# achiever04/face-recognition-platform

Hardware: AMD Instinct MI355X
Metric: faces/sec (detect+embed+match) on 1080p @ 100k gallery (higher is better)
Workload: dtype f16; 1 GPU; 32x1080x1920 BGR frames per GPU per step resident in HBM, host results out every step, 2 batches in flight per GPU (one handle = one stream each, used round-robin), forced K=10 faces/frame, 100000-identity fp16 gallery, FRPDet detector fp16 + ArcFace IResNet-100 fp16 (synthetic seeded weights); batch_frames=32, faces_per_frame=10, gallery=100000, streams=1, lanes=2, lane_warmup_steps=20

## Files before the change

face-recognition-platform_amd/csrc/conv_mfma.hip:

```cpp
#include <hip/hip_runtime.h>
#include <stdint.h>
#include <stdlib.h>
#include <type_traits>
#include "frp_internal.h"
#include "conv_common.h"

namespace frp {

template <int TP, int TC, int WP, int WC, int NS, int NW, bool SMALL>
__global__ __launch_bounds__(NW * 64, TP == 128 ? 4 : 2) void conv_mfma_kernel(ConvParams p_in) {
    extern __shared__ __attribute__((aligned(16))) unsigned char smem[];
    ConvParams p = p_in;
    if (p.n_dev) {
        int n = *p.n_dev;
        n = n < 0 ? 0 : (n > p.N ? p.N : n);
        p.M = n * p.Ho * p.Wo;
        p.n_ptiles = (p.M + TP - 1) / TP;
        if (p.ksplit < 0) p.ksplit = conv_pick_ksplit(p.M, p.Cout, p.Ktot, p.flags, p.res != nullptr, p.n_cu);
    }
    constexpr int XB = TP * 128;
    constexpr int WB = TC * 128;
    constexpr int STAGE = XB + WB;
    constexpr int XI = TP / 8 / NW;
    constexpr int WI = TC / 8 / NW;
// ... 340 lines not shown
        attr_set[dev] = true;
    }
    const int ncu = device_cu_count(dev);
    if (ncu <= 0) return hipErrorInvalidDevice;
    const int ks_grid = p.ksplit < 0 ? conv_pick_ksplit(p.Ho * p.Wo, p.Cout, p.Ktot, p.flags, p.res != nullptr, ncu) : p.ksplit;
    const long ntiles = (long)p.n_ptiles * p.n_ctiles * ks_grid;
    if (ntiles <= 0 || ntiles > 0x7fffffffL) return hipErrorInvalidValue;
    p.n_cu = ncu;
    const long slots = (long)ncu * (lds <= 80 * 1024 ? 2 : 1);
    unsigned grid = (unsigned)(ntiles < slots ? ntiles : slots);
    p.n_workers = 0;
    if (TP == 128 && p.pf_ptr && p.pf_bytes >= 4096 && grid <= 128 && (long)grid + CONV_PF_WGS <= slots) {
        p.n_workers = (int)grid;
        grid += CONV_PF_WGS;
    }
    if (grid > 256) p.stamps = nullptr;
    hipLaunchKernelGGL(kern, dim3(grid), dim3(NW * 64), lds, stream, p);
    return hipGetLastError();
}

hipError_t launch_conv(const ConvParams& in, hipStream_t stream) {
    ConvParams p = in;
    if (!(p.KS == 1 || p.KS == 3) || !(p.stride == 1 || p.stride == 2)) return hipErrorInvalidValue;
    if (p.Cin < 8 || (p.Cin & 7) || (p.Cout & 7) || p.N <= 0 || p.H <= 0 || p.W <= 0) return hipErrorInvalidValue;
    p.pad = p.KS / 2;
    p.Ho = (p.H + 2 * p.pad - p.KS) / p.stride + 1;
    p.Wo = (p.W + 2 * p.pad - p.KS) / p.stride + 1;
    const long M = (long)p.N * p.Ho * p.Wo;
    if (M <= 0 || M > 0x7fffffffL) return hipErrorInvalidValue;
    p.M = (int)M;
    p.Ktot = p.KS * p.KS * p.Cin;
    p.x2_bytes = 0;
    p.x2_shift = 0;
    if (p.x2) {
        if (p.KS != 3 || (p.Cin & 63) || p.Cin2 <= 0 || (p.Cin2 & 63) || !(p.Cin == p.Cin2 || p.Cin == 2 * p.Cin2) || p.ksplit > 1 ||
            (p.flags & (FRP_FLAG_F8 | FRP_FLAG_BORDER_BIAS)) || p.wino_w)
            return hipErrorInvalidValue;
        const long x2b = (long)p.N * p.H * p.W * p.Cin2 * 2;
        if (x2b >= 0x7fffffffL) return hipErrorInvalidValue;
        p.x2_bytes = (unsigned)x2b;
        p.x2_shift = p.Cin == p.Cin2 ? 0 : 1;
        p.Ktot += p.Cin2;
    }
    p.nk = (p.Ktot + 63) / 64;
    if (p.ksplit < 0 && !(p.n_dev && (p.flags & FRP_FLAG_OUT_F32) && !p.res && !(p.Cin & 63))) return hipErrorInvalidValue;
    if (p.ksplit == 0) p.ksplit = 1;
    if (p.ksplit > 1 && (p.nk % p.ksplit != 0 || !(p.flags & FRP_FLAG_OUT_F32) || p.res || (p.Cin & 63)))
        return hipErrorInvalidValue;
    const bool f8 = (p.flags & FRP_FLAG_F8) != 0;
    const int es = f8 ? 1 : 2;
    const long xb = (long)p.N * p.H * p.W * p.Cin * es, wb = (long)p.Cout * p.Ktot * es;
    if (xb >= 0x7fffffffL || wb >= 0x7fffffffL) return hipErrorInvalidValue;
    if ((p.flags & FRP_FLAG_OUT_FP8) && !f8) return hipErrorInvalidValue;
    if ((p.out2 || f8) && ((p.flags & FRP_FLAG_OUT_F32) || p.ksplit != 1 || !(p.out_scale > 0.f))) return hipErrorInvalidValue;
    p.x_bytes = (unsigned)xb;
    p.w_bytes = (unsigned)wb;
    const bool small = (p.Cin & 63) != 0;
    p.cin_shift = 0;
    if (small) {
        if (p.Cin & (p.Cin - 1)) return hipErrorInvalidValue;
        while ((1 << p.cin_shift) < p.Cin) ++p.cin_shift;
    }
    if ((p.flags & FRP_FLAG_BORDER_BIAS) && !(p.KS == 3 && p.stride == 1 && p.Ho >= 2 && p.Wo >= 2))
        return hipErrorInvalidValue;
    if ((p.flags & FRP_FLAG_RES_UP2) && (!p.res || p.Hr * 2 != p.Ho || p.Wr * 2 != p.Wo)) return hipErrorInvalidValue;
    if (!p.x || !p.w || !p.bias || !p.out) return hipErrorInvalidValue;
    if (p.act == FRP_ACT_PRELU && !p.slope) return hipErrorInvalidValue;
    if (f8) {
        if (!conv3x3_rows_eligible(p) || (p.Cin & 127) || !p.wscale || !(p.in_scale > 0.f)) return hipErrorInvalidValue;
        return launch_conv3x3_lean(p, stream);
    }
    int ncu_ = p.n_cu;
    if (ncu_ <= 0) {
        int dev_ = 0;
        if (hipGetDevice(&dev_) != hipSuccess || dev_ < 0 || dev_ >= 64) return hipErrorInvalidDevice;
        ncu_ = device_cu_count(dev_);
    }
    const bool few = conv_small_m(p, (long)((p.M + 255) / 256) * ((p.Cout + 127) / 128), ncu_);
    if (p.wino_w && !p.x2 && !(p.dbg & CONV_DBG_GENERIC) && conv3x3_wino_eligible(p)) {
        p.w = p.wino_w;
        return launch_conv3x3_wino(p, stream);
    }
    if ((p.dbg & CONV_DBG_S2) && !(p.dbg & CONV_DBG_GENERIC) && !few && conv3x3_s2_eligible(p)) return launch_conv3x3_s2(p, stream);
    if (p.stem_x) return (p.small_m <= 0 && conv3x3_c64_eligible(p)) ? launch_conv3x3_c64(p, stream) : hipErrorInvalidValue;
    if (!(p.dbg & (CONV_DBG_GENERIC | CONV_DBG_NO_C64)) && p.small_m <= 0 && conv3x3_c64_eligible(p)) return launch_conv3x3_c64(p, stream);
#ifdef FRP_LAB
    if (!(p.dbg & CONV_DBG_GENERIC) && !p.x2 && conv3x3_rows_eligible(p)) return launch_conv3x3_rows(p, stream);
#else
    if (!(p.dbg & CONV_DBG_GENERIC) && !p.x2 && conv3x3_rows_eligible(p)) return launch_conv3x3_lean(p, stream);
#endif
    if (!small && few) return launch_cfg<128, 64, 4, 2, 3, 8, false>(p, stream);
    if (p.Cout > 64)
        return small ? launch_cfg<256, 128, 4, 2, 3, 8, true>(p, stream) : launch_cfg<256, 128, 4, 2, 3, 8, false>(p, stream);
    return small ? launch_cfg<256, 64, 8, 1, 3, 8, true>(p, stream) : launch_cfg<256, 64, 8, 1, 3, 8, false>(p, stream);
}

}
```

face-recognition-platform_amd/csrc/frp_api.cpp:

```cpp
#include <hip/hip_runtime.h>
#include <rccl/rccl.h>
#include <dlfcn.h>

#include <algorithm>
#include <cmath>
#include <cstdio>
#include <cstdlib>
#include <cstring>
#include <mutex>
#include <string>
#include <vector>
#include <thread>
#include <atomic>

#include "frp.h"
#ifdef FRP_LAB
#include "frp_lab.h"
#endif
#include "frp_blob.h"
#include "frp_internal.h"
#include "jpeg_host.h"

using namespace frp;

#define FRP_WINO_MIN_FACES 128
Switches frp::read_switches() {
    auto set = [](const char* n) { return getenv(n) ? 1 : 0; };
    const char *sm = getenv("FRP_SMALL_M"), *wm = getenv("FRP_WINO_MIN_FACES");
    Switches s{};
    s.small_m = !sm ? 0 : (sm[0] == '0' ? -1 : 1);
    s.wino_min_faces = wm ? atoi(wm) : FRP_WINO_MIN_FACES;
    s.s2 = set("FRP_S2"); s.host_count = set("FRP_HOST_COUNT"); s.match_v1 = set("FRP_MATCH_V1");
    s.no_fused_stem12 = set("FRP_NO_FUSED_STEM12"); s.no_fused_stem = set("FRP_NO_FUSED_STEM");
    s.no_emb_stem = set("FRP_NO_EMB_STEM"); s.no_stem_fuse = set("FRP_NO_STEM_FUSE");
    s.no_wino = set("FRP_NO_WINO"); s.no_kconcat = set("FRP_NO_KCONCAT");
    return s;
}

const ProcessSwitches& frp::process_switches() {
    static const ProcessSwitches s = [] {
        const char* jh = getenv("FRP_JPEG_DEVICE_HUFFMAN");
        return ProcessSwitches{getenv("FRP_NO_GRAPH") != nullptr, getenv("FRP_C64_ALL") != nullptr, !jh ? 0 : (jh[0] == '0' ? -1 : 1)};
    }();
    return s;
}

namespace {

struct DevBuf {
    void* p = nullptr;
    size_t cap = 0;
};

struct TensorDims {
    int h = 0, w = 0, c = 0;
    bool f32 = false;
    bool f8 = false;
};

struct Net {
    std::vector<frp_conv_op> ops;
    int n_bufs = 0;
    int in_buf = 0, in_ch = 0;
    std::vector<DevBuf> bufs;
    std::vector<TensorDims> dims;
    std::vector<int64_t> wino_off;
    std::vector<int> kc_skip;
    std::vector<int> kc_src;
    std::vector<int64_t> kc_w_off, kc_bias_off;
};

enum { EV_START = 0, EV_H2D, EV_PRE, EV_DET, EV_DEC, EV_ALIGN, EV_EMB, EV_L2, EV_MATCH, EV_D2H, EV_COUNT };

struct NetGraph {
    std::string key;
    hipGraphExec_t exec = nullptr;
    uint64_t epoch = 0;
    double dflops = 0, df8flops = 0;
    int64_t dlaunches = 0, df8launches = 0;
    int fc_ksplit = 0, fc_ktot = 0;
    const float* fc_bias = nullptr;
    std::vector<TensorDims> dims;
};

}

struct frp_handle {
    int device = 0;
    hipStream_t stream = nullptr;
    std::mutex mu;
    std::string err;
    frp_config cfg{};
    bool have_weights = false;
    frp_blob_header hdr{};
    DevBuf wdata;
    Net det, emb;
    DevBuf frames;
    int rB = 0, rH = 0, rW = 0;
    int n_cu = 256;
    DevBuf frames_next;
    int nB = 0, nH = 0, nW = 0;
    bool next_valid = false;
    hipStream_t copy_stream = nullptr;
    hipEvent_t ev_next_ready = nullptr, ev_next_free = nullptr;
    std::vector<void*> pinned;
    DevBuf scaled;
    int dH = 0, dW = 0;
    bool det_scaled = false;
    int canvas_h = 0, canvas_w = 0;
    int det_op_limit = -1;
    std::vector<NetGraph> graphs;
    std::vector<std::string> graph_seen, graph_bad;
    uint64_t alloc_epoch = 1;
    int64_t graph_replays = 0;
    void* comm = nullptr;
    int dist_rank = 0, dist_world = 0;
    DevBuf det_hashes;
    bool det_hash_on = false;
// ... 175 lines not shown
    return (float)std::log((double)t / (1.0 - (double)t));
}

void rec(frp_handle* h, int which) {
    if (h->cfg.profile) (void)hipEventRecord(h->ev[which], h->stream);
}

int plan_net(frp_handle* h, Net& net, int batch, int H, int W, bool skip_input = false) {
    net.dims.assign(net.n_bufs, TensorDims());
    std::vector<size_t> need(net.n_bufs, 0);
    net.dims[net.in_buf] = {H, W, net.in_ch, false};
    need[net.in_buf] = skip_input ? 0 : (size_t)batch * H * W * net.in_ch * 2;
    for (const frp_conv_op& op : net.ops) {
        TensorDims in = net.dims[op.in_buf];
        if (in.c == 0) return fail(h, FRP_ERR_BLOB, "program reads an unwritten buffer");
        if (op.flags & FRP_FLAG_FLATTEN) in = {1, 1, in.h * in.w * in.c, false};
        if (in.c != op.cin) return fail(h, FRP_ERR_BLOB, "program channel mismatch");
        const int pad = op.ksize / 2;
        TensorDims out;
        out.h = (in.h + 2 * pad - op.ksize) / op.stride + 1;
        out.w = (in.w + 2 * pad - op.ksize) / op.stride + 1;
        out.c = op.cout;
        out.f32 = (op.flags & FRP_FLAG_OUT_F32) != 0;
        if (out.h <= 0 || out.w <= 0) return fail(h, FRP_ERR_INVALID, "input too small for the network");
        if (in.f32) return fail(h, FRP_ERR_BLOB, "program reads an fp32 tensor as a conv input");
        const bool op_f8 = (op.flags & FRP_OPFLAG_FP8_MFMA) != 0;
        if (in.f8 != op_f8) return fail(h, FRP_ERR_BLOB, "program operand precision mismatch (fp8 op <-> fp8 tensor)");
        if (op_f8 && !(op.ksize == 3 && op.stride == 1 && (op.cin & 127) == 0 && !(op.flags & (FRP_FLAG_OUT_F32 | FRP_FLAG_FLATTEN | FRP_FLAG_RES_UP2))))
            return fail(h, FRP_ERR_BLOB, "op shape not covered by the fp8 matrix path");
        out.f8 = (op.flags & FRP_OPFLAG_OUT_FP8) != 0;
        if (out.f8 && (out.f32 || !op_f8)) return fail(h, FRP_ERR_BLOB, "fp8 primary output needs an fp8 op");
        if (op.res_buf >= 0) {
            const TensorDims& r = net.dims[op.res_buf];
            const bool up2 = (op.flags & FRP_FLAG_RES_UP2) != 0;
            if (r.c != op.cout || r.f32 || r.f8 || (up2 ? (r.h * 2 != out.h || r.w * 2 != out.w) : (r.h != out.h || r.w != out.w)))
                return fail(h, FRP_ERR_BLOB, "program residual shape mismatch");
        }
        net.dims[op.out_buf] = out;
        need[op.out_buf] = std::max(need[op.out_buf], (size_t)batch * out.h * out.w * out.c * (out.f32 ? 4 : out.f8 ? 1 : 2));
        if (op.out2_buf >= 0) {
            if (out.f32 || out.f8) return fail(h, FRP_ERR_BLOB, "fp8 copy of a non-fp16 output");
            TensorDims o2 = out;
            o2.f8 = true;
            net.dims[op.out2_buf] = o2;
            need[op.out2_buf] = std::max(need[op.out2_buf], (size_t)batch * out.h * out.w * out.c);
        }
    }
    for (int i = 0; i < net.n_bufs; ++i)
        if (need[i]) FRPCHK(ensure(h, net.bufs[i], need[i]));
    return FRP_OK;
}

bool stem_fusable(const Net& net) {
    if (net.ops.empty()) return false;
    const frp_conv_op& op = net.ops[0];
    return op.in_buf == net.in_buf && op.cin == 8 && op.cout == 32 && op.ksize == 3 && op.stride == 2 &&
           op.act == FRP_ACT_RELU && op.res_buf < 0 && (op.flags & ~0) == 0 && (op.real_ch & 0xffff) == 3;
}

bool stem12_fusable(const Net& net) {
    if (!stem_fusable(net) || net.ops.size() < 2) return false;
    const frp_conv_op& a = net.ops[0];
    const frp_conv_op& b = net.ops[1];
    if (!(b.in_buf == a.out_buf && b.cin == 32 && b.cout == 64 && b.ksize == 3 && b.stride == 2 && b.act == FRP_ACT_RELU &&
          b.res_buf < 0 && b.flags == 0))
        return false;
    for (size_t i = 2; i < net.ops.size(); ++i)
        if (net.ops[i].in_buf == a.out_buf || net.ops[i].res_buf == a.out_buf) {
            bool rewritten = false;
            for (size_t j = 2; j < i; ++j) rewritten |= net.ops[j].out_buf == a.out_buf;
            if (!rewritten) return false;
        }
    return true;
}

int run_net_body(frp_handle* h, const Switches& sw, Net& net, int batch, int H, int W, double* flops, int64_t* launches, const StemParams* stem,
                 const int32_t* n_dev, bool allow_wino) {
    std::vector<TensorDims> d(net.n_bufs);
    d[net.in_buf] = {H, W, net.in_ch, false};
    const char* wbase = (const char*)h->wdata.p;
    bool first = true;
    size_t skip = 0;
    if (&net == &h->det && h->det_hash_on) HIPCHK(h, hipMemsetAsync(h->det_hashes.p, 0, 64 * 8, h->stream));
    const int dbg = (sw.s2 ? CONV_DBG_S2 : 0) | (process_switches().c64_all ? CONV_DBG_C64_ALL : 0);
    if (stem && stem12_fusable(net) && (stem->Hc % 4) == 0 && (stem->Wc % 4) == 0 && !sw.no_fused_stem12) {
        const frp_conv_op& a = net.ops[0];
        const frp_conv_op& b = net.ops[1];
        Stem12Params sp{};
        sp.frames = stem->frames; sp.B = stem->B; sp.H = stem->H; sp.W = stem->W;
        sp.row_stride = stem->row_stride; sp.frame_stride = stem->frame_stride;
        sp.Hc = stem->Hc; sp.Wc = stem->Wc; sp.Ho1 = stem->Hc / 2; sp.Wo1 = stem->Wc / 2; sp.Ho2 = stem->Hc / 4; sp.Wo2 = stem->Wc / 4;
        sp.rgb_in = stem->rgb_in;
        sp.w1 = (const _Float16*)(wbase + a.w_off); sp.bias1 = (const float*)(wbase + a.bias_off);
        sp.w2 = (const _Float16*)(wbase + b.w_off); sp.bias2 = (const float*)(wbase + b.bias_off);
        sp.out = (_Float16*)net.bufs[b.out_buf].p;
        hipError_t e = launch_stem12_u8(sp, h->stream);
        if (e != hipSuccess) return fail(h, FRP_ERR_HIP, std::string("launch_stem12_u8: ") + hipGetErrorString(e));
        d[a.out_buf] = {sp.Ho1, sp.Wo1, 32, false};
        d[b.out_buf] = {sp.Ho2, sp.Wo2, 64, false};
        *flops += 2.0 * batch * sp.Ho1 * sp.Wo1 * 9.0 * 3 * 32 + 2.0 * batch * sp.Ho2 * sp.Wo2 * 9.0 * 32 * 64;
        *launches += 1;
        if (h->det_hash_on) {
            e = launch_tensor_hash(sp.out, (size_t)batch * sp.Ho2 * sp.Wo2 * 64 * 2, (unsigned long long*)h->det_hashes.p + 1, h->stream);
            if (e != hipSuccess) return fail(h, FRP_ERR_HIP, std::string("tensor_hash: ") + hipGetErrorString(e));
        }
        skip = 2;
        first = false;
    }
    bool fuse_stem = false, fuse_even_only = false;
    size_t fuse_op = 0;
    EmbStemParams fused{};
    if (!stem && !net.ops.empty()) {
        const frp_conv_op& a = net.ops[0];
        if (a.in_buf == net.in_buf && a.cin == 8 && (a.real_ch & 0xffff) == 3 && a.cout == 64 && a.ksize == 3 && a.stride == 1 &&
            a.act == FRP_ACT_PRELU && a.res_buf < 0 && a.flags == 0 && a.slope_off >= 0 && !sw.no_emb_stem) {
            EmbStemParams ep{};
            ep.x = (const _Float16*)net.bufs[a.in_buf].p;
            ep.M = batch; ep.H = H; ep.W = W;
            ep.w = (const _Float16*)(wbase + a.w_off);
            ep.bias = (const float*)(wbase + a.bias_off);
            ep.slope = (const float*)(wbase + a.slope_off);
            ep.out = (_Float16*)net.bufs[a.out_buf].p;
            ep.n_dev = n_dev;
            size_t nb = 1;
            while (nb < net.ops.size() && nb < net.kc_skip.size() && net.kc_skip[nb]) ++nb;
            if (nb < net.ops.size() && !sw.no_stem_fuse && sw.small_m <= 0) {
                const frp_conv_op& b = net.ops[nb];
                const bool plain = !(b.flags & ~FRP_FLAG_BORDER_BIAS) && (b.flags & FRP_FLAG_BORDER_BIAS) && b.out2_buf < 0 && b.res_buf < 0;
                const bool chained = !(nb < net.kc_src.size() && net.kc_src[nb] >= 0);
                fuse_stem = plain && chained && b.in_buf == a.out_buf && b.out_buf != a.out_buf && b.out_buf != a.in_buf && a.out_buf != a.in_buf && b.cin == 64 && b.cout == 64 && b.ksize == 3 &&
                            b.stride == 1 && b.act == FRP_ACT_PRELU && b.slope_off >= 0 && conv3x3_c64_fuses_stem(batch, H, W, h->n_cu);
                fuse_op = nb;
                fuse_even_only = true;
                for (size_t j = 1; j < net.ops.size(); ++j) {
                    const frp_conv_op& o = net.ops[j];
                    if (j == nb || (o.in_buf != a.out_buf && o.res_buf != a.out_buf)) continue;
                    const bool shortcut = j < net.kc_skip.size() && net.kc_skip[j] && o.in_buf == a.out_buf && o.res_buf != a.out_buf &&
                                          o.ksize == 1 && o.stride == 2;
                    if (!shortcut) fuse_even_only = false;
                }
            }
            if (fuse_stem) {
                fused = ep;
            } else {
                hipError_t e = launch_emb_stem(ep, h->stream);
                if (e != hipSuccess) return fail(h, FRP_ERR_HIP, std::string("launch_emb_stem: ") + hipGetErrorString(e));
                *launches += 1;
            }
            d[a.out_buf] = {H, W, 64, false};
            *flops += 2.0 * batch * H * W * 9.0 * 3 * 64;
            skip = 1;
            first = false;
        }
    }
    for (const frp_conv_op& op : net.ops) {
        if (&net == &h->det && h->det_op_limit >= 0 && (int)(&op - net.ops.data()) >= h->det_op_limit) break;
        if (skip) { --skip; continue; }
        if (first && stem) {
            first = false;
            StemParams sp = *stem;
            sp.w = (const _Float16*)(wbase + op.w_off);
            sp.bias = (const float*)(wbase + op.bias_off);
            sp.out = (_Float16*)net.bufs[op.out_buf].p;
            hipError_t e = launch_stem_u8(sp, h->stream);
            if (e != hipSuccess) return fail(h, FRP_ERR_HIP, std::string("launch_stem_u8: ") + hipGetErrorString(e));
            d[op.out_buf] = {sp.Ho, sp.Wo, 32, false};
            *flops += 2.0 * batch * sp.Ho * sp.Wo * 9.0 * 3 * 32;
// ... 1745 lines not shown
    HIPCHK(h, hipMemcpyAsync(h->scratch.p, chips, (size_t)M * FRP_CHIP_PIX * 3, hipMemcpyHostToDevice, h->stream));
    hipError_t e = launch_chips_to_blob((const uint8_t*)h->scratch.p, M, (_Float16*)h->emb.bufs[h->emb.in_buf].p, h->stream);
    if (e != hipSuccess) return fail(h, FRP_ERR_HIP, std::string("chips_to_blob: ") + hipGetErrorString(e));
    FRPCHK(run_embed(h, read_switches(), M));
    HIPCHK(h, hipMemcpyAsync(emb, h->emb.bufs[h->hdr.emb_out_buf].p, (size_t)M * FRP_EMB_DIM * 4, hipMemcpyDeviceToHost, h->stream));
    HIPCHK(h, hipStreamSynchronize(h->stream));
    return FRP_OK;
}

static int match_common(frp_handle* h, const float* q, int M, float* all_scores_host, int32_t* idx, float* cos) {
    const Switches sw = read_switches();
    if (!q || M <= 0 || M > (1 << 20)) return fail(h, FRP_ERR_INVALID, "bad query arguments");
    if (h->g_rows <= 0) return fail(h, FRP_ERR_NO_GALLERY, "gallery is empty");
    const int mpad = round_up(M, 32);
    FRPCHK(ensure(h, h->q16, (size_t)mpad * FRP_EMB_DIM * 2));
    HIPCHK(h, hipMemsetAsync(h->q16.p, 0, (size_t)mpad * FRP_EMB_DIM * 2, h->stream));
    FRPCHK(upload_rows_normalized(h, q, M, (_Float16*)h->q16.p));
    DevBuf all;
    if (all_scores_host) FRPCHK(ensure(h, all, (size_t)M * h->g_rows * 4));
    int rc = run_match(h, sw, M, (float*)all.p);
    hipError_t e = hipSuccess;
    if (rc == FRP_OK) {
        if (idx) e = hipMemcpyAsync(idx, h->best_idx.p, (size_t)M * 4, hipMemcpyDeviceToHost, h->stream);
        if (e == hipSuccess && cos) e = hipMemcpyAsync(cos, h->best_cos.p, (size_t)M * 4, hipMemcpyDeviceToHost, h->stream);
        if (e == hipSuccess && all_scores_host)
            e = hipMemcpyAsync(all_scores_host, all.p, (size_t)M * h->g_rows * 4, hipMemcpyDeviceToHost, h->stream);
    }
    hipError_t e2 = hipStreamSynchronize(h->stream);
    release(all);
    if (rc != FRP_OK) return rc;
    if (e != hipSuccess || e2 != hipSuccess) return fail(h, FRP_ERR_HIP, "match result copy failed");
    return FRP_OK;
}

int frp_match(frp_handle* h, const float* q, int32_t M, int32_t topk, int32_t* idx, float* cos) {
    if (!h) return FRP_ERR_INVALID;
    Guard g(h);
    if (topk < 1 || topk > FRP_MAX_TOPK) return fail(h, FRP_ERR_INVALID, "topk must be in 1..FRP_MAX_TOPK");
    if (topk == 1) return match_common(h, q, M, nullptr, idx, cos);
    if (!q || !idx || !cos || M <= 0 || M > (1 << 20)) return fail(h, FRP_ERR_INVALID, "bad query arguments");
    if (h->g_rows <= 0) return fail(h, FRP_ERR_NO_GALLERY, "gallery is empty");
    const long N = h->g_rows;
    const Switches sw = read_switches();
    int chunk = (int)std::max<long>(1, std::min<long>(M, (1L << 28) / N));
    DevBuf all, didx, dcos;
    int rc = ensure(h, all, (size_t)chunk * N * 4);
    if (rc == FRP_OK) rc = ensure(h, didx, (size_t)chunk * topk * 4);
    if (rc == FRP_OK) rc = ensure(h, dcos, (size_t)chunk * topk * 4);
    hipError_t e = hipSuccess;
    for (int m0 = 0; rc == FRP_OK && e == hipSuccess && m0 < M; m0 += chunk) {
        const int m = std::min(chunk, M - m0);
        const int mpad = round_up(m, 32);
        rc = ensure(h, h->q16, (size_t)mpad * FRP_EMB_DIM * 2);
        if (rc != FRP_OK) break;
        e = hipMemsetAsync(h->q16.p, 0, (size_t)mpad * FRP_EMB_DIM * 2, h->stream);
        if (e != hipSuccess) break;
        rc = upload_rows_normalized(h, q + (size_t)m0 * FRP_EMB_DIM, m, (_Float16*)h->q16.p);
        if (rc == FRP_OK) rc = run_match(h, sw, m, (float*)all.p);
        if (rc != FRP_OK) break;
        e = launch_topk_rows((const float*)all.p, m, N, topk, (int32_t*)didx.p, (float*)dcos.p, h->stream);
        if (e == hipSuccess) e = hipMemcpyAsync(idx + (size_t)m0 * topk, didx.p, (size_t)m * topk * 4, hipMemcpyDeviceToHost, h->stream);
        if (e == hipSuccess) e = hipMemcpyAsync(cos + (size_t)m0 * topk, dcos.p, (size_t)m * topk * 4, hipMemcpyDeviceToHost, h->stream);
        if (e == hipSuccess) e = hipStreamSynchronize(h->stream);
    }
    (void)hipStreamSynchronize(h->stream);
    release(all); release(didx); release(dcos);
    if (rc != FRP_OK) return rc;
    if (e != hipSuccess) return fail(h, FRP_ERR_HIP, std::string("match top-k: ") + hipGetErrorString(e));
    return FRP_OK;
}

int frp_match_scores(frp_handle* h, const float* q, int32_t M, float* cos_all, int64_t n_cols) {
    if (!h) return FRP_ERR_INVALID;
    Guard g(h);
    if (!cos_all) return fail(h, FRP_ERR_INVALID, "null output");
    if (n_cols != h->g_rows) return fail(h, FRP_ERR_INVALID, "match_scores: output sized for another gallery size");
    return match_common(h, q, M, cos_all, nullptr, nullptr);
}

namespace {
void conv_route_from_abi_flags(int32_t flags, ConvParams& p) {
    p.dbg = ((flags >> 8) & 0xff) | ((flags & (1 << 19)) ? CONV_DBG_WINO_2D : 0) | ((flags & (1 << 20)) ? CONV_DBG_NO_C64 : 0) |
            ((flags & (1 << 21)) ? CONV_DBG_S2 : 0) | ((flags & (1 << 22)) ? CONV_DBG_C64_SAME_ORDER : 0) |
            (process_switches().c64_all ? CONV_DBG_C64_ALL : 0);
    p.small_m = (flags & (1 << 17)) ? 1 : (flags & ((1 << 18) | (1 << 16))) ? -1 : 0;
}
}

int frp_conv2d_nhwc(frp_handle* h, const void* x, int32_t N, int32_t H, int32_t W, int32_t Cin, const void* w, int32_t Cout,
                    int32_t ksize, int32_t stride, const float* bias, const float* slope, const void* res, int32_t res_h,
                    int32_t res_w, int32_t act, int32_t flags, void* out) {
    if (!h) return FRP_ERR_INVALID;
    Guard g(h);
    if (!x || !w || !bias || !out || N <= 0 || H <= 0 || W <= 0 || Cin <= 0 || Cout <= 0 || !(ksize == 1 || ksize == 3) ||
        !(stride == 1 || stride == 2))
        return fail(h, FRP_ERR_INVALID, "bad conv arguments");
    const int pad = ksize / 2;
    const int Ho = (H + 2 * pad - ksize) / stride + 1, Wo = (W + 2 * pad - ksize) / stride + 1;
    const bool up2 = flags & FRP_FLAG_RES_UP2;
    const size_t xb = (size_t)N * H * W * Cin * 2, wb = (size_t)Cout * ksize * ksize * Cin * 2;
    const size_t bb = (size_t)Cout * 4 * ((flags & FRP_FLAG_BORDER_BIAS) ? 9 : 1);
    const size_t ob = (size_t)N * Ho * Wo * Cout * ((flags & FRP_FLAG_OUT_F32) ? 4 : 2);
    const size_t rb = res ? (size_t)N * (up2 ? res_h : Ho) * (up2 ? res_w : Wo) * Cout * 2 : 0;
    DevBuf dx, dw, db, ds, dr, dout, dwino;
    int rc = ensure(h, dx, xb);
    if (rc == FRP_OK) rc = ensure(h, dw, wb);
    if (rc == FRP_OK) rc = ensure(h, db, bb);
    if (rc == FRP_OK) rc = ensure(h, dout, ob);
    if (rc == FRP_OK && slope) rc = ensure(h, ds, (size_t)Cout * 4);
    if (rc == FRP_OK && res) rc = ensure(h, dr, rb);
    ConvParams p{};
    conv_route_from_abi_flags(flags, p);
    const bool want_wino = (flags & (1 << 16)) != 0;
    std::vector<uint16_t> wimg;
    if (want_wino) {
        bool shape_ok = conv3x3_wino_shape_ok(W, Cin, ksize, stride) ||
                        (ksize == 3 && stride == 1 && conv3x3_wino_wide_pays(N, H, W, Cin, Cout, h->n_cu, res != nullptr));
#ifdef FRP_LAB
        shape_ok = shape_ok || ((p.dbg & (CONV_DBG_WINO_ROW_PATCH | CONV_DBG_WINO_2D)) && conv3x3_wino_lab_shape_ok(W, Cin, ksize, stride));
#endif
        if (!shape_ok || (flags & (FRP_FLAG_OUT_F32 | FRP_FLAG_RES_UP2)))
            return fail(h, FRP_ERR_INVALID, "shape not covered by the Winograd kernel");
        wimg.resize(conv3x3_wino_image_bytes(Cin, Cout) / 2);
        build_wino_image((const uint16_t*)w, Cin, Cout, wimg.data());
        if (rc == FRP_OK) rc = ensure(h, dwino, wimg.size() * 2);
    }
    hipError_t e = hipSuccess;
    if (rc == FRP_OK) {
        e = hipMemcpyAsync(dx.p, x, xb, hipMemcpyHostToDevice, h->stream);
        if (e == hipSuccess && want_wino) e = hipMemcpyAsync(dwino.p, wimg.data(), wimg.size() * 2, hipMemcpyHostToDevice, h->stream);
        if (e == hipSuccess) e = hipMemcpyAsync(dw.p, w, wb, hipMemcpyHostToDevice, h->stream);
        if (e == hipSuccess) e = hipMemcpyAsync(db.p, bias, bb, hipMemcpyHostToDevice, h->stream);
        if (e == hipSuccess && slope) e = hipMemcpyAsync(ds.p, slope, (size_t)Cout * 4, hipMemcpyHostToDevice, h->stream);
        if (e == hipSuccess && res) e = hipMemcpyAsync(dr.p, res, rb, hipMemcpyHostToDevice, h->stream);
        if (e == hipSuccess) {
            p.x = (const _Float16*)dx.p; p.w = (const _Float16*)dw.p; p.bias = (const float*)db.p;
            p.slope = slope ? (const float*)ds.p : nullptr;
            p.res = res ? (const _Float16*)dr.p : nullptr;
            p.out = dout.p;
            p.N = N; p.H = H; p.W = W; p.Cin = Cin; p.Cout = Cout; p.KS = ksize; p.stride = stride; p.act = act;
            p.flags = flags & (FRP_FLAG_BORDER_BIAS | FRP_FLAG_OUT_F32 | FRP_FLAG_RES_UP2);
            p.Hr = res_h; p.Wr = res_w;
            if (want_wino) p.wino_w = (const _Float16*)dwino.p;
            e = launch_conv(p, h->stream);
        }
        if (e == hipSuccess) e = hipMemcpyAsync(out, dout.p, ob, hipMemcpyDeviceToHost, h->stream);
    }
    hipError_t e2 = hipStreamSynchronize(h->stream);
    DevBuf* all[] = {&dx, &dw, &db, &ds, &dr, &dout, &dwino};
    for (DevBuf* b : all) release(*b);
    if (rc != FRP_OK) return rc;
    if (e != hipSuccess) return fail(h, e == hipErrorInvalidValue ? FRP_ERR_INVALID : FRP_ERR_HIP, std::string("conv2d: ") + hipGetErrorString(e));
    if (e2 != hipSuccess) return fail(h, FRP_ERR_HIP, std::string("conv2d sync: ") + hipGetErrorString(e2));
    return FRP_OK;
}

int frp_conv2d_f8(frp_handle* h, const void* x8, int32_t N, int32_t H, int32_t W, int32_t Cin, const void* w8, int32_t Cout,
                  const float* wscale, const float* bias, const float* slope, const void* res16, int32_t act, int32_t flags,
                  float in_scale, float out_scale, void* out, void* out2_f8) {
    if (!h) return FRP_ERR_INVALID;
    Guard g(h);
    if (!x8 || !w8 || !wscale || !bias || !out || N <= 0 || H <= 0 || W <= 0 || Cin <= 0 || Cout <= 0)
        return fail(h, FRP_ERR_INVALID, "bad conv arguments");
    const bool out8 = (flags & FRP_FLAG_OUT_FP8) != 0;
    const size_t xb = (size_t)N * H * W * Cin, wb = (size_t)Cout * 9 * Cin, on = (size_t)N * H * W * Cout;
    const size_t bb = (size_t)Cout * 4 * ((flags & FRP_FLAG_BORDER_BIAS) ? 9 : 1);
// ... 208 lines not shown
```

face-recognition-platform_amd/csrc/frp_internal.h:

```cpp
#pragma once
#include <hip/hip_runtime.h>
#include <stdint.h>
#include <type_traits>

#define FRP_ACT_NONE 0
#define FRP_ACT_RELU 1
#define FRP_ACT_PRELU 2
#define FRP_FLAG_BORDER_BIAS 1
#define FRP_FLAG_OUT_F32 2
#define FRP_FLAG_RES_UP2 4
#define FRP_FLAG_FLATTEN 8
#define FRP_FLAG_F8 32
#define FRP_FLAG_OUT_FP8 64
#define FRP_CHIP_PIX (112 * 112)
#ifndef FRP_MAX_FACES_CAP
#define FRP_MAX_FACES_CAP 128
#endif

#include "jpeg_host.h"

namespace frp {

struct Switches {
    int small_m;
    int s2;
    int no_fused_stem12;
    int no_fused_stem;
    int no_emb_stem;
    int no_stem_fuse;
    int wino_min_faces;
    int host_count;
    int match_v1;
    int no_wino;
    int no_kconcat;
};
static_assert(std::has_unique_object_representations_v<Switches>, "run_net keys captured graphs by the bytes of a Switches");
Switches read_switches();

struct ProcessSwitches {
    bool no_graph;
    bool c64_all;
    int jpeg_device_huffman;
};
const ProcessSwitches& process_switches();

struct ConvParams {
    const _Float16* x;
    const _Float16* w;
    const float* bias;
    const float* slope;
    const _Float16* res;
    void* out;
    void* out2;
    const _Float16* x2;
    int Cin2;
    const float* wscale;
    float in_scale;
    float out_scale;
    int N, H, W, Cin, Cout, KS, stride;
    int act, flags;
    int Hr, Wr;
    int ksplit;
    const _Float16* wino_w;
    const int32_t* n_dev;
    int n_cu;
    unsigned long long* stamps;
    int dbg;
    int wino_wide_only;
    const void* pf_ptr;
    unsigned pf_bytes;
    int n_workers;
    int small_m;
    const _Float16* stem_x;
    const _Float16* stem_w;
    const float* stem_bias;
    const float* stem_slope;
    _Float16* stem_out;
    int stem_even_only;
    int pad, Ho, Wo, M, Ktot, nk, cin_shift, n_ptiles, n_ctiles;
    unsigned x_bytes, w_bytes, x2_bytes;
    int x2_shift;
};

constexpr int CONV_DBG_GENERIC = 1;
constexpr int CONV_DBG_WINO_2D = 256;
constexpr int CONV_DBG_NO_C64 = 512;
constexpr int CONV_DBG_C64_ALL = 1024;
constexpr int CONV_DBG_S2 = 2048;
constexpr int CONV_DBG_C64_SAME_ORDER = 4096;
constexpr int CONV_DBG_LEAN_ALL_ROWS = 64;
constexpr int CONV_DBG_LEAN_TILE256 = 128;
constexpr int CONV_DBG_WINO_ABLATION = 15 << 1;
constexpr int CONV_DBG_WINO_ONE_WAVE = 32;
constexpr int CONV_DBG_WINO_ROW_PATCH = 64;
constexpr int CONV_DBG_WINO_KLOOP_GEN1 = 128;
constexpr int CONV_DBG_ROWS_PRE_PREFETCH = 2;
constexpr int CONV_DBG_ROWS_ABLATION = 15 << 2;
constexpr int CONV_DBG_ROWS_GEN1 = 64;
constexpr int CONV_DBG_ROUTING = CONV_DBG_GENERIC | CONV_DBG_WINO_2D | CONV_DBG_NO_C64 | CONV_DBG_C64_ALL | CONV_DBG_S2 | CONV_DBG_C64_SAME_ORDER;
template <class... B> constexpr bool conv_dbg_disjoint(B... b) { return (b + ...) == (b | ...); }
static_assert(conv_dbg_disjoint(CONV_DBG_GENERIC, CONV_DBG_WINO_2D, CONV_DBG_NO_C64, CONV_DBG_C64_ALL, CONV_DBG_S2, CONV_DBG_C64_SAME_ORDER) &&
              conv_dbg_disjoint(CONV_DBG_ROUTING, CONV_DBG_LEAN_ALL_ROWS, CONV_DBG_LEAN_TILE256) &&
              conv_dbg_disjoint(CONV_DBG_ROUTING, CONV_DBG_WINO_ABLATION, CONV_DBG_WINO_ONE_WAVE, CONV_DBG_WINO_ROW_PATCH, CONV_DBG_WINO_KLOOP_GEN1) &&
              conv_dbg_disjoint(CONV_DBG_ROUTING, CONV_DBG_ROWS_PRE_PREFETCH, CONV_DBG_ROWS_ABLATION, CONV_DBG_ROWS_GEN1),
              "the dbg bits one kernel family reads must be disjoint");
constexpr int conv_dbg_field(int dbg, int field) { return (dbg & field) / (field & -field); }

hipError_t launch_conv(const ConvParams& p, hipStream_t stream);
bool conv3x3_rows_eligible(const ConvParams& p);
#ifdef FRP_LAB
hipError_t launch_conv3x3_rows(const ConvParams& p, hipStream_t stream);
#endif
hipError_t launch_conv3x3_lean(const ConvParams& p, hipStream_t stream);
bool conv3x3_c64_eligible(const ConvParams& p);
bool conv3x3_c64_fuses_stem(int N, int H, int W, int n_cu);
hipError_t launch_conv3x3_c64(const ConvParams& p, hipStream_t stream);
bool conv3x3_s2_eligible(const ConvParams& p);
hipError_t launch_conv3x3_s2(const ConvParams& p, hipStream_t stream);
bool conv3x3_wino_eligible(const ConvParams& p);
bool conv3x3_wino_shape_ok(int W, int Cin, int ksize, int stride);
bool conv3x3_wino_wide_pays(int N, int H, int W, int Cin, int Cout, int n_cu, bool has_res);
#ifdef FRP_LAB
bool conv3x3_wino_lab_shape_ok(int W, int Cin, int ksize, int stride);
#endif
size_t conv3x3_wino_image_bytes(int Cin, int Cout);
hipError_t launch_conv3x3_wino(const ConvParams& p, hipStream_t stream);

hipError_t launch_preprocess(const uint8_t* bgr, int B, int H, int W, long row_stride, long frame_stride,
                             _Float16* out, int Hc, int Wc, int rgb_in, hipStream_t stream);

struct StemParams {
    const uint8_t* frames;
    int B, H, W;
    long row_stride, frame_stride;
    int Hc, Wc;
    int Ho, Wo;
    int rgb_in;
    const _Float16* w;
    const float* bias;
    _Float16* out;
};
hipError_t launch_stem_u8(const StemParams& p, hipStream_t stream);

struct Stem12Params {
    const uint8_t* frames;
    int B, H, W;
    long row_stride, frame_stride;
    int Hc, Wc;
    int Ho1, Wo1;
    int Ho2, Wo2;
    int rgb_in;
    const _Float16* w1;
    const float* bias1;
    const _Float16* w2;
    const float* bias2;
    _Float16* out;
};
hipError_t launch_stem12_u8(const Stem12Params& p, hipStream_t stream);

struct EmbStemParams {
    const _Float16* x;
    int M, H, W;
    const _Float16* w;
    const float* bias;
    const float* slope;
    _Float16* out;
    const int32_t* n_dev;
};
hipError_t launch_emb_stem(const EmbStemParams& p, hipStream_t stream);

struct DecodeParams {
    const _Float16* head[3];
    int hl[3], wl[3];
    int B, max_faces;
    float logit_thresh, nms_iou;
    float* boxes;
    float* kps;
    float* scores;
    int32_t* anchor;
    int32_t* counts;
    _Float16* logits;
};
hipError_t launch_decode_nms(const DecodeParams& p, hipStream_t stream);

struct JpegParams {
    const int16_t* coef;
    const uint16_t* qtab;
    uint8_t* planes;
    uint8_t* frames;
    int B, W, H, components;
    int bx[3], by[3];
    int blocks_per_image;
    long plane_off[3], plane_img;
    int hs, vs;
    int cw, ch;
};
hipError_t launch_jpeg_decode(const JpegParams& p, hipStream_t stream);

struct JpegHuffParams {
    const uint8_t* scan;
    const uint32_t* int_off;
// ... 78 lines not shown
```

Before: 28120 faces/s.

## Add persistent lean kernel for stride-2 3x3 convolutions with LDS DMA pipeline

Adds a dedicated persistent kernel for stride-2, pad-1 3x3 convolutions. It uses a three-stage LDS ring filled by buffer-load-to-LDS DMA, interleaved with MFMA groups, and prefetches the next tile's descriptors and bias/slope while the current tile computes. The kernel is routed by default for eligible non-small, non-few shapes, replacing the generic implicit-GEMM path for these layers, with an env switch to disable it. Risks include correctness of the tap and residual-concat tail ordering and lower occupancy from the large LDS footprint.

```diff
diff --git a/face-recognition-platform_amd/csrc/conv3x3_s2lean.hip b/face-recognition-platform_amd/csrc/conv3x3_s2lean.hip
--- /dev/null
+++ b/face-recognition-platform_amd/csrc/conv3x3_s2lean.hip
@@ -0,0 +1,365 @@
+#include <hip/hip_runtime.h>
+#include <stdint.h>
+#include "frp_internal.h"
+#include "conv_common.h"
+
+namespace frp {
+
+namespace {
+__device__ __forceinline__ void s2l_dma(__amdgpu_buffer_rsrc_t rsrc, unsigned char* lds_base, unsigned voffset, int soffset) {
+    __builtin_amdgcn_raw_ptr_buffer_load_lds(rsrc, (__attribute__((address_space(3))) void*)lds_base, 16, voffset, soffset, 0, 0);
+}
+__device__ __forceinline__ __amdgpu_buffer_rsrc_t s2l_rsrc(const void* ptr, unsigned bytes) {
+    return __builtin_amdgcn_make_buffer_rsrc(const_cast<void*>(ptr), 0, bytes, 0x00020000);
+}
+__device__ __forceinline__ void s2l_fence() { __builtin_amdgcn_sched_barrier(0); }
+}
+
+template <int TC, int WP, int WC>
+__global__ __launch_bounds__(512, 2) void conv3x3_s2lean_kernel(ConvParams p_in) {
+    extern __shared__ __attribute__((aligned(256))) unsigned char smem[];
+    ConvParams p = p_in;
+    constexpr int TP = 256, NW = 8;
+    if (p.n_dev) {
+        int n = *p.n_dev;
+        n = n < 0 ? 0 : (n > p.N ? p.N : n);
+        p.M = n * p.Ho * p.Wo;
+        p.n_ptiles = (p.M + TP - 1) / TP;
+    }
+    constexpr int XB = TP * 128;
+    constexpr int WB = TC * 128;
+    constexpr int STAGE = XB + WB;
+    constexpr int XI = TP / 8 / NW;
+    constexpr int WI = TC / 8 / NW;
+    constexpr int LPS = XI + WI;
+    constexpr int MP = TP / WP / 32, MC = TC / WC / 32;
+    constexpr int OFF_PAR = 3 * STAGE;
+    constexpr int PAR = 10 * TC * 4;
+    static_assert(WP * WC == NW && XI == 4 && (WI == 1 || WI == 2) && MP * MC <= 4, "tile/wave layout");
+
+    const int t = threadIdx.x;
+    const int lane = t & 63;
+    const int wave = __builtin_amdgcn_readfirstlane(t >> 6);
+
+    const int n_tiles = p.n_ptiles * p.n_ctiles;
+    const int G = (int)gridDim.x;
+    int t0, t1, tstep;
+    if ((G & 7) == 0) {
+        const int x = blockIdx.x & 7, j = blockIdx.x >> 3, per = G >> 3;
+        const int cs = (int)((long)x * n_tiles / 8), ce = (int)((long)(x + 1) * n_tiles / 8);
+        t0 = cs + j;
+        t1 = ce;
+        tstep = per;
+    } else {
+        t0 = (int)((long)blockIdx.x * n_tiles / G);
+        t1 = (int)((long)(blockIdx.x + 1) * n_tiles / G);
+        tstep = 1;
+    }
+    if (t0 >= t1) return;
+
+    const __amdgpu_buffer_rsrc_t xrsrc = s2l_rsrc(p.x, p.x_bytes);
+    const __amdgpu_buffer_rsrc_t wrsrc = s2l_rsrc(p.w, p.w_bytes);
+    const void* x2ptr = p.x2 ? (const void*)p.x2 : (const void*)p.x;
+    const unsigned x2bytes = p.x2 ? p.x2_bytes : 0u;
+
+    const int cpt = p.Cin >> 6;
+    const int c2 = p.x2 ? (p.Cin2 >> 6) : 0;
+    const int cin2b = p.Cin * 2;
+    const int rowpitch = p.W * cin2b;
+    const int x2tap = (p.W + 1) * p.Cin2 * 2;
+
+    int lrow = lane >> 3;
+    const int lchunk = (lane & 7) ^ (((wave & 1) << 2) | (lane >> 4));
+    const int lch16 = lchunk * 16;
+    const int HoWo = p.Ho * p.Wo;
+    const float inv_howo = 1.0f / (float)HoWo, inv_wo = 1.0f / (float)p.Wo;
+
+    struct Desc { int xoff[XI]; unsigned mask[XI]; unsigned woff[WI]; };
+    auto make_desc = [&](int tile, Desc& d) {
+        const bool live = tile < t1;
+        const int ptile = tile / p.n_ctiles;
+        const int m0i = ptile * TP;
+        const int c0i = (tile - ptile * p.n_ctiles) * TC;
+#pragma unroll
+        for (int i = 0; i < XI; ++i) {
+            const int m = m0i + (i * NW + wave) * 8 + lrow;
+            unsigned mask = 0;
+            int off = 0;
+            if (live && m < p.M) {
+                int n, rem, oy, ox;
+                fast_divmod(m, HoWo, inv_howo, n, rem);
+                fast_divmod(rem, p.Wo, inv_wo, oy, ox);
+                const int y0 = oy * 2 - 1, x0 = ox * 2 - 1;
+                off = (((n * p.H + y0) * p.W + x0) * p.Cin) * 2;
+                unsigned ym = 0, xm = 0;
+#pragma unroll
+                for (int dd = 0; dd < 3; ++dd) {
+                    ym |= ((unsigned)(y0 + dd) < (unsigned)p.H ? 1u : 0u) << dd;
+                    xm |= ((unsigned)(x0 + dd) < (unsigned)p.W ? 1u : 0u) << dd;
+                }
+#pragma unroll
+                for (int dd = 0; dd < 3; ++dd) mask |= ((ym >> dd) & 1u) ? (xm << (3 * dd)) : 0u;
+            }
+            d.xoff[i] = off;
+            d.mask[i] = mask;
+        }
+#pragma unroll
+        for (int i = 0; i < WI; ++i) {
+            const int co = c0i + (i * NW + wave) * 8 + lrow;
+            d.woff[i] = (live && co < p.Cout) ? (unsigned)(co * p.Ktot * 2 + lch16) : CONV_OOB;
+        }
+    };
+
+    struct Follow {
+        const void* ptr; unsigned bytes;
+        int xo[XI]; unsigned mk[XI]; unsigned wo[WI];
+        int s_off;
+        unsigned bit;
+        int wadd;
+    };
+    Desc cur, nt;
+    struct Tail { bool s2; const void* ptr; unsigned bytes; int s_off; unsigned bit; int wadd; };
+    auto tail = [&](int q) -> Tail {
+        Tail r;
+        r.s2 = q < c2;
+        const int tp = q - c2;
+        r.ptr = r.s2 ? x2ptr : (const void*)p.x;
+        r.bytes = r.s2 ? x2bytes : p.x_bytes;
+        r.s_off = r.s2 ? x2tap + (q << 7) : tp * cin2b;
+        r.bit = r.s2 ? 16u : (1u << tp);
+        r.wadd = r.s2 ? ((9 * cpt + q) << 7) : ((tp * cpt) << 7);
+        return r;
+    };
+    auto fill = [&](bool inner, const Tail& tl, int in_soff, unsigned in_bit, int in_wadd, Follow& f) __attribute__((always_inline)) {
+        const bool s2 = !inner && tl.s2;
+        const bool own = inner || tl.s2;
+        f.ptr = inner ? (const void*)p.x : tl.ptr;
+        f.bytes = inner ? p.x_bytes : tl.bytes;
+#pragma unroll
+        for (int i = 0; i < XI; ++i) {
+            const int sh = cur.xoff[i] >> p.x2_shift, cx = cur.xoff[i], nx = nt.xoff[i];
+            const unsigned cm = cur.mask[i], nm = nt.mask[i];
+            f.xo[i] = s2 ? sh : own ? cx : nx;
+            f.mk[i] = own ? cm : nm;
+        }
+#pragma unroll
+        for (int i = 0; i < WI; ++i) {
+            const unsigned cw = cur.woff[i], nw = nt.woff[i];
+            f.wo[i] = own ? cw : nw;
+        }
+        f.s_off = inner ? in_soff : tl.s_off;
+        f.bit = inner ? in_bit : tl.bit;
+        f.wadd = inner ? in_wadd : tl.wadd;
+    };
+
+    const int wave_p = wave / WC, wave_c = wave - wave_p * WC;
+    const int prow0 = wave_p * (TP / WP), crow0 = wave_c * (TC / WC);
+    const int fr = lane & 31, fh = lane >> 5;
+    int pvx[MP], pwa[MC];
+#pragma unroll
+    for (int i = 0; i < MP; ++i) pvx[i] = lds_off(prow0 + i * 32 + fr, fh);
+#pragma unroll
+    for (int j = 0; j < MC; ++j) pwa[j] = XB + lds_off(crow0 + j * 32 + fr, fh);
+
+    floatx16 acc[MP][MC];
+    half8 bf[2][MP], af[2][MC];
+
+    constexpr int PPT = (9 * TC + NW * 64 - 1) / (NW * 64);
+    float pb[PPT], ps = 0.f;
+    int t_e = t, fr_e = lane & 31, fh_e = lane >> 5;
+    const bool border_ = p.flags & FRP_FLAG_BORDER_BIAS;
+    auto fetch_params = [&](int tile) {
+        const int c0p = (tile % p.n_ctiles) * TC;
+        const int nb = (border_ ? 9 : 1) * TC;
+#pragma unroll
+        for (int q = 0; q < PPT; ++q) {
+            const int idx = t_e + q * NW * 64;
+            const int cls = idx / TC, co = c0p + (idx - cls * TC);
+            pb[q] = (idx < nb && co < p.Cout) ? p.bias[(long)cls * p.Cout + co] : 0.f;
+        }
+        if (p.act == FRP_ACT_PRELU && t_e < TC) ps = (c0p + t_e < p.Cout) ? p.slope[c0p + t_e] : 0.f;
+    };
+    auto store_params = [&](int par) {
+        float* lb = reinterpret_cast<float*>(smem + OFF_PAR + par * PAR);
+#pragma unroll
+        for (int q = 0; q < PPT; ++q) {
+            const int idx = t + q * NW * 64;
+            if (idx < 9 * TC) lb[idx] = pb[q];
+        }
+        if (t < TC) lb[9 * TC + t] = ps;
+    };
+
+    auto step = [&](int rd, int is, __amdgpu_buffer_rsrc_t xr, const unsigned (&xv)[XI], const unsigned (&wv)[WI], int wadd)
+                    __attribute__((always_inline)) {
+        wait_vmcnt<LPS>();
+        retire_lds_reads();
+        __builtin_amdgcn_s_barrier();
+        asm volatile("" : "+s"(rd));
+        auto read_frags = [&](int kk, int S) {
+#pragma unroll
+            for (int i = 0; i < MP; ++i) bf[S][i] = *reinterpret_cast<const half8*>(smem + (rd + (pvx[i] ^ (kk << 5))));
+#pragma unroll
+            for (int j = 0; j < MC; ++j) af[S][j] = *reinterpret_cast<const half8*>(smem + (rd + (pwa[j] ^ (kk << 5))));
+        };
+        auto mfma_group = [&](int S) {
+#pragma unroll
+            for (int i = 0; i < MP; ++i)
+#pragma unroll
+                for (int j = 0; j < MC; ++j)
+                    acc[i][j] = __builtin_amdgcn_mfma_f32_32x32x16_f16(af[S][j], bf[S][i], acc[i][j], 0, 0, 0);
+        };
+        unsigned char* xd = smem + is + wave * 1024;
+        unsigned char* wd = xd + XB;
+        read_frags(0, 0);
+        read_frags(1, 1);
+        s2l_fence();
+        mfma_group(0);
+#pragma unroll
+        for (int i = 0; i < WI; ++i) s2l_dma(wrsrc, wd + i * NW * 1024, wv[i], wadd);
+        read_frags(2, 0);
+        s2l_fence();
+        mfma_group(1);
+        s2l_dma(xr, xd, xv[0], 0);
+        s2l_dma(xr, xd + NW * 1024, xv[1], 0);
+        read_frags(3, 1);
+        s2l_fence();
+        mfma_group(0);
+        s2l_dma(xr, xd + 2 * NW * 1024, xv[2], 0);
+        s2l_dma(xr, xd + 3 * NW * 1024, xv[3], 0);
+        s2l_fence();
+        mfma_group(1);
+        s2l_fence();
+    };
+    auto follow_step = [&](int rd, int is, const Follow& f) __attribute__((always_inline)) {
+        unsigned xv[XI];
+#pragma unroll
+        for (int i = 0; i < XI; ++i) xv[i] = (f.mk[i] & f.bit) ? (unsigned)(f.xo[i] + f.s_off + lch16) : CONV_OOB;
+        step(rd, is, s2l_rsrc(f.ptr, f.bytes), xv, f.wo, f.wadd);
+    };
+
+    make_desc(t0, cur);
+#pragma unroll
+    for (int s = 0; s < 2; ++s) {
+#pragma unroll
+        for (int i = 0; i < XI; ++i)
+            s2l_dma(xrsrc, smem + s * STAGE + (i * NW + wave) * 1024,
+                    (cur.mask[i] & (1u << s)) ? (unsigned)(cur.xoff[i] + s * cin2b + lch16) : CONV_OOB, 0);
+#pragma unroll
+        for (int i = 0; i < WI; ++i) s2l_dma(wrsrc, smem + s * STAGE + XB + (i * NW + wave) * 1024, cur.woff[i], (s * cpt) << 7);
+    }
+    fetch_params(t0);
+    store_params(0);
+    int r0 = 0, r1 = STAGE, r2 = 2 * STAGE;
+    int par = 0;
+    const bool has_res = p.res != nullptr;
+
+    for (int ct = t0; ct < t1; ct += tstep) {
+#pragma unroll
+        for (int i = 0; i < MP; ++i)
+#pragma unroll
+            for (int j = 0; j < MC; ++j)
+#pragma unroll
+                for (int e = 0; e < 16; ++e) acc[i][j][e] = 0.f;
+        asm volatile("" : "+v"(t_e), "+v"(fr_e), "+v"(fh_e), "+v"(lrow));
+        make_desc(ct + tstep, nt);
+        wait_vmcnt<0>();
+        fetch_params(ct + tstep);
+
+#define S2L_STEP(TAP)                                                                                               \
+    do {                                                                                                            \
+        constexpr int T2 = (TAP) + 2;                                                                               \
+        const int so_ = (T2 / 3) * rowpitch + (T2 % 3) * cin2b + cbs;                                               \
+        unsigned xv_[XI];                                                                                           \
+        _Pragma("unroll") for (int i = 0; i < XI; ++i)                                                              \
+            xv_[i] = (cur.mask[i] & (1u << T2)) ? (unsigned)(cur.xoff[i] + so_ + lch16) : CONV_OOB;                 \
+        step((TAP) % 3 == 0 ? r0 : (TAP) % 3 == 1 ? r1 : r2, T2 % 3 == 0 ? r0 : T2 % 3 == 1 ? r1 : r2, xrsrc, xv_,  \
+             cur.woff, (T2 * cpt + cb) << 7);                                                                       \
+    } while (0)
+
+        const Tail tl0 = tail(0), tl1 = tail(1);
+        for (int cb = 0; cb < cpt; ++cb) {
+            const int cbs = cb << 7;
+            const bool inner = cb + 1 < cpt;
+            S2L_STEP(0);
+            S2L_STEP(1);
+            S2L_STEP(2);
+            S2L_STEP(3);
+            S2L_STEP(4);
+            S2L_STEP(5);
+            S2L_STEP(6);
+            Follow fa, fb;
+            fill(inner, tl0, cbs + 128, 1u, (cb + 1) << 7, fa);
+            fill(inner, tl1, cin2b + cbs + 128, 2u, (cpt + cb + 1) << 7, fb);
+            follow_step(r1, r0, fa);
+            follow_step(r2, r1, fb);
+        }
+#undef S2L_STEP
+        for (int j = 0; j < c2; ++j) {
+            Follow f;
+            fill(false, tail(j + 2), 0, 0u, 0, f);
+            follow_step(r0, r2, f);
+            const int r_ = r0;
+            r0 = r1;
+            r1 = r2;
+            r2 = r_;
+        }
+
+        store_params(par ^ 1);
+        const int ptile = ct / p.n_ctiles;
+        const int m0 = ptile * TP;
+        const int c0 = (ct - ptile * p.n_ctiles) * TC;
+        {
+            const float* lds_bias = reinterpret_cast<const float*>(smem + OFF_PAR + par * PAR);
+            const float* lds_slope = lds_bias + 9 * TC;
+            uint4 rres[MP][MC][2];
+            if (has_res) conv_residual_loads<MP, MC>(p, rres, m0, c0, prow0, crow0, fr_e, fh_e, HoWo, inv_howo, inv_wo);
+            conv_epilogue<MP, MC, TC>(p, acc, rres, lds_bias, lds_slope, m0, c0, TP, prow0, crow0, fr_e, fh_e, HoWo, inv_howo, inv_wo);
+        }
+        par ^= 1;
+        cur = nt;
+    }
+    wait_vmcnt<0>();
+}
+
+template <int TC, int WP, int WC>
+static hipError_t launch_s2lean_cfg(const ConvParams& p0, hipStream_t stream) {
+    ConvParams p = p0;
+    constexpr int TP = 256;
+    p.n_ptiles = (p.M + TP - 1) / TP;
+    p.n_ctiles = (p.Cout + TC - 1) / TC;
+    const int lds = 3 * (TP + TC) * 128 + 2 * 10 * TC * 4;
+    static bool attr_set[64] = {};
+    auto kern = conv3x3_s2lean_kernel<TC, WP, WC>;
+    int dev = 0;
+    if (hipGetDevice(&dev) != hipSuccess || dev < 0 || dev >= 64) return hipErrorInvalidDevice;
+    if (!attr_set[dev]) {
+        hipError_t e = hipFuncSetAttribute(reinterpret_cast<const void*>(kern), hipFuncAttributeMaxDynamicSharedMemorySize, lds);
+        if (e != hipSuccess) return e;
+        attr_set[dev] = true;
+    }
+    const int ncu = device_cu_count(dev);
+    if (ncu <= 0) return hipErrorInvalidDevice;
+    const long ntiles = (long)p.n_ptiles * p.n_ctiles;
+    if (ntiles <= 0 || ntiles > 0x7fffffffL) return hipErrorInvalidValue;
+    p.n_cu = ncu;
+    p.n_workers = 0;
+    p.stamps = nullptr;
+    const unsigned grid = (unsigned)(ntiles < ncu ? ntiles : ncu);
+    hipLaunchKernelGGL(kern, dim3(grid), dim3(512), lds, stream, p);
+    return hipGetLastError();
+}
+
+bool conv3x3_s2lean_eligible(const ConvParams& p) {
+    if (p.KS != 3 || p.stride != 2 || p.pad != 1 || (p.Cin & 63) || p.Cin < 64 || p.ksplit != 1) return false;
+    if ((p.flags & (FRP_FLAG_F8 | FRP_FLAG_OUT_FP8 | FRP_FLAG_BORDER_BIAS)) || p.out2 || p.stem_x || p.wino_w) return false;
+    if (p.x2 && (p.Cin2 <= 0 || (p.Cin2 & 63))) return false;
+    return true;
+}
+
+hipError_t launch_conv3x3_s2lean(const ConvParams& p, hipStream_t stream) {
+    if (!conv3x3_s2lean_eligible(p)) return hipErrorInvalidValue;
+    if (p.Cout > 64) return launch_s2lean_cfg<128, 4, 2>(p, stream);
+    return launch_s2lean_cfg<64, 8, 1>(p, stream);
+}
+
+}
diff --git a/face-recognition-platform_amd/csrc/conv_mfma.hip b/face-recognition-platform_amd/csrc/conv_mfma.hip
--- a/face-recognition-platform_amd/csrc/conv_mfma.hip
+++ b/face-recognition-platform_amd/csrc/conv_mfma.hip
@@ -446,6 +446,7 @@
         return launch_conv3x3_wino(p, stream);
     }
     if ((p.dbg & CONV_DBG_S2) && !(p.dbg & CONV_DBG_GENERIC) && !few && conv3x3_s2_eligible(p)) return launch_conv3x3_s2(p, stream);
+    if (!(p.dbg & (CONV_DBG_GENERIC | CONV_DBG_NO_S2_STATIC)) && !few && !small && conv3x3_s2lean_eligible(p)) return launch_conv3x3_s2lean(p, stream);
     if (p.stem_x) return (p.small_m <= 0 && conv3x3_c64_eligible(p)) ? launch_conv3x3_c64(p, stream) : hipErrorInvalidValue;
     if (!(p.dbg & (CONV_DBG_GENERIC | CONV_DBG_NO_C64)) && p.small_m <= 0 && conv3x3_c64_eligible(p)) return launch_conv3x3_c64(p, stream);
 #ifdef FRP_LAB
diff --git a/face-recognition-platform_amd/csrc/frp_api.cpp b/face-recognition-platform_amd/csrc/frp_api.cpp
--- a/face-recognition-platform_amd/csrc/frp_api.cpp
+++ b/face-recognition-platform_amd/csrc/frp_api.cpp
@@ -34,6 +34,7 @@
     s.no_fused_stem12 = set("FRP_NO_FUSED_STEM12"); s.no_fused_stem = set("FRP_NO_FUSED_STEM");
     s.no_emb_stem = set("FRP_NO_EMB_STEM"); s.no_stem_fuse = set("FRP_NO_STEM_FUSE");
     s.no_wino = set("FRP_NO_WINO"); s.no_kconcat = set("FRP_NO_KCONCAT");
+    s.no_s2_static = set("FRP_NO_S2_STATIC");
     return s;
 }
 
@@ -375,7 +376,7 @@
     bool first = true;
     size_t skip = 0;
     if (&net == &h->det && h->det_hash_on) HIPCHK(h, hipMemsetAsync(h->det_hashes.p, 0, 64 * 8, h->stream));
-    const int dbg = (sw.s2 ? CONV_DBG_S2 : 0) | (process_switches().c64_all ? CONV_DBG_C64_ALL : 0);
+    const int dbg = (sw.s2 ? CONV_DBG_S2 : 0) | (sw.no_s2_static ? CONV_DBG_NO_S2_STATIC : 0) | (process_switches().c64_all ? CONV_DBG_C64_ALL : 0);
     if (stem && stem12_fusable(net) && (stem->Hc % 4) == 0 && (stem->Wc % 4) == 0 && !sw.no_fused_stem12) {
         const frp_conv_op& a = net.ops[0];
         const frp_conv_op& b = net.ops[1];
@@ -2287,6 +2288,7 @@
 void conv_route_from_abi_flags(int32_t flags, ConvParams& p) {
     p.dbg = ((flags >> 8) & 0xff) | ((flags & (1 << 19)) ? CONV_DBG_WINO_2D : 0) | ((flags & (1 << 20)) ? CONV_DBG_NO_C64 : 0) |
             ((flags & (1 << 21)) ? CONV_DBG_S2 : 0) | ((flags & (1 << 22)) ? CONV_DBG_C64_SAME_ORDER : 0) |
+            ((flags & (1 << 23)) ? CONV_DBG_NO_S2_STATIC : 0) |
             (process_switches().c64_all ? CONV_DBG_C64_ALL : 0);
     p.small_m = (flags & (1 << 17)) ? 1 : (flags & ((1 << 18) | (1 << 16))) ? -1 : 0;
 }
diff --git a/face-recognition-platform_amd/csrc/frp_internal.h b/face-recognition-platform_amd/csrc/frp_internal.h
--- a/face-recognition-platform_amd/csrc/frp_internal.h
+++ b/face-recognition-platform_amd/csrc/frp_internal.h
@@ -24,6 +24,7 @@
 struct Switches {
     int small_m;
     int s2;
+    int no_s2_static;
     int no_fused_stem12;
     int no_fused_stem;
     int no_emb_stem;
@@ -88,6 +89,7 @@
 constexpr int CONV_DBG_C64_ALL = 1024;
 constexpr int CONV_DBG_S2 = 2048;
 constexpr int CONV_DBG_C64_SAME_ORDER = 4096;
+constexpr int CONV_DBG_NO_S2_STATIC = 8192;
 constexpr int CONV_DBG_LEAN_ALL_ROWS = 64;
 constexpr int CONV_DBG_LEAN_TILE256 = 128;
 constexpr int CONV_DBG_WINO_ABLATION = 15 << 1;
@@ -97,9 +99,11 @@
 constexpr int CONV_DBG_ROWS_PRE_PREFETCH = 2;
 constexpr int CONV_DBG_ROWS_ABLATION = 15 << 2;
 constexpr int CONV_DBG_ROWS_GEN1 = 64;
-constexpr int CONV_DBG_ROUTING = CONV_DBG_GENERIC | CONV_DBG_WINO_2D | CONV_DBG_NO_C64 | CONV_DBG_C64_ALL | CONV_DBG_S2 | CONV_DBG_C64_SAME_ORDER;
+constexpr int CONV_DBG_ROUTING = CONV_DBG_GENERIC | CONV_DBG_WINO_2D | CONV_DBG_NO_C64 | CONV_DBG_C64_ALL | CONV_DBG_S2 | CONV_DBG_C64_SAME_ORDER |
+                                 CONV_DBG_NO_S2_STATIC;
 template <class... B> constexpr bool conv_dbg_disjoint(B... b) { return (b + ...) == (b | ...); }
-static_assert(conv_dbg_disjoint(CONV_DBG_GENERIC, CONV_DBG_WINO_2D, CONV_DBG_NO_C64, CONV_DBG_C64_ALL, CONV_DBG_S2, CONV_DBG_C64_SAME_ORDER) &&
+static_assert(conv_dbg_disjoint(CONV_DBG_GENERIC, CONV_DBG_WINO_2D, CONV_DBG_NO_C64, CONV_DBG_C64_ALL, CONV_DBG_S2, CONV_DBG_C64_SAME_ORDER,
+                                CONV_DBG_NO_S2_STATIC) &&
               conv_dbg_disjoint(CONV_DBG_ROUTING, CONV_DBG_LEAN_ALL_ROWS, CONV_DBG_LEAN_TILE256) &&
               conv_dbg_disjoint(CONV_DBG_ROUTING, CONV_DBG_WINO_ABLATION, CONV_DBG_WINO_ONE_WAVE, CONV_DBG_WINO_ROW_PATCH, CONV_DBG_WINO_KLOOP_GEN1) &&
               conv_dbg_disjoint(CONV_DBG_ROUTING, CONV_DBG_ROWS_PRE_PREFETCH, CONV_DBG_ROWS_ABLATION, CONV_DBG_ROWS_GEN1),
@@ -117,6 +121,8 @@
 hipError_t launch_conv3x3_c64(const ConvParams& p, hipStream_t stream);
 bool conv3x3_s2_eligible(const ConvParams& p);
 hipError_t launch_conv3x3_s2(const ConvParams& p, hipStream_t stream);
+bool conv3x3_s2lean_eligible(const ConvParams& p);
+hipError_t launch_conv3x3_s2lean(const ConvParams& p, hipStream_t stream);
 bool conv3x3_wino_eligible(const ConvParams& p);
 bool conv3x3_wino_shape_ok(int W, int Cin, int ksize, int stride);
 bool conv3x3_wino_wide_pays(int N, int H, int W, int Cin, int Cout, int n_cu, bool has_res);
```

Result: no change. 28310 faces/s (median of 6 runs) (+0.7%).
